# hooman007/ProtoASNet

Hardware: NVIDIA B200
Metric: head_fwd_clips_per_sec (higher is better)
Workload: dtype bf16

## Files before the change

### protoasnet_b200/csrc/head_sm100.cu

```cuda
#include <cstdlib>

#include "head_sm100_shared.cuh"

namespace pasn {
using namespace sm100;

using namespace k1;

namespace {
constexpr int K2_THREADS = 320;
constexpr uint32_t K2_STAGE = 65536;
constexpr uint32_t K2_SM_V = 2 * K2_STAGE;
constexpr uint32_t K2_V_BYTES = PP_MAX * 257 * 4;
constexpr uint32_t K2_SM_MISC = K2_SM_V + 49408;
constexpr uint32_t K2_SM_ORD = K2_SM_MISC + 8192;
constexpr int K2_MAX_ORD = 4096;
constexpr uint32_t K2_SMEM = K2_SM_ORD + 2 * K2_MAX_ORD;

struct K2Params {
  const uint8_t* feimg; const float* osum; const uint8_t* packed; size_t off_w2, off_b2;
  const float* protos; const float* last_layer;
  float* logits; float* sim; float* dist; float* feats;
  const int64_t* labels; const int32_t* proto_class; long long global_offset; unsigned long long* best_key;
  const int* ready;
  int cpc, grid1;
  int* queue;
  int* tile_owner;
  int a_kmajor, l2_hints;
  float* stash;
  int N, P, PP, K, cpt, ntiles;
  int* err;
  int* fault;
  long long* trace;
};
__device__ __forceinline__ long long gtimer_ns() {
  long long t;
  asm volatile("mov.u64 %0, %%globaltimer;" : "=l"(t));
  return t;
}
}
#define K2_TRACE(slot) do { if (p.trace != nullptr && blockIdx.x == 0 && (slot) < 184) p.trace[768 + 16 + (slot)] = gtimer_ns(); } while (0)

__global__ void __launch_bounds__(K2_THREADS, 1) proto_w2_kernel(const K2Params p) {
  extern __shared__ __align__(1024) unsigned char smem[];
  uint64_t* bars = reinterpret_cast<uint64_t*>(smem + K2_SM_MISC);
  uint32_t* tmem_ptr_s = reinterpret_cast<uint32_t*>(smem + K2_SM_MISC + 64);
  volatile int* abort_s = reinterpret_cast<volatile int*>(smem + K2_SM_MISC + 72);
  float* s_vn = reinterpret_cast<float*>(smem + K2_SM_MISC + 128);
  float* s_b2 = reinterpret_cast<float*>(smem + K2_SM_MISC + 512);
  float* s_part = reinterpret_cast<float*>(smem + K2_SM_MISC + 1536);
  float* s_sim = reinterpret_cast<float*>(smem + K2_SM_MISC + 3584);
  unsigned long long* s_key = reinterpret_cast<unsigned long long*>(smem + K2_SM_MISC + 4608);
  uint64_t* tbars = reinterpret_cast<uint64_t*>(smem + K2_SM_MISC + 5632);
  volatile int* s_tile = reinterpret_cast<volatile int*>(smem + K2_SM_MISC + 5696);
  int* s_win = reinterpret_cast<int*>(smem + K2_SM_MISC + 5120);
  float* s_v = reinterpret_cast<float*>(smem + K2_SM_V);

  const int tid = threadIdx.x, warp = tid >> 5, lane = tid & 31;
  Ctx ctx{p.err, abort_s, p.fault, 0};
  if ((smem_u32(smem) & 1023u) != 0) {
    if (tid == 0) atomicCAS(p.err, 0, 901);
    return;
  }
  if (tid == 0) K2_TRACE(0);
  if (tid == 0) {
    *abort_s = 0;
    mbar_init(&bars[0], 1); mbar_init(&bars[1], 1); mbar_init(&bars[2], 1); mbar_init(&bars[3], 1);
    mbar_init(&bars[4], 1); mbar_init(&bars[5], 1); mbar_init(&bars[6], 8); mbar_init(&bars[7], 8);
    for (int i = 0; i < 4; ++i) mbar_init(&tbars[i], 1);
    fence_mbar_init();
  }
  if (warp == 0) tmem_alloc(tmem_ptr_s, 512);
  for (int i = tid; i < DD; i += K2_THREADS) s_b2[i] = reinterpret_cast<const float*>(p.packed + p.off_b2)[i];
  if (tid < p.P) s_key[tid] = p.stash ? (p.best_key[tid] ^ PASN_KEY_SIGN) : PASN_KEY_NONE;
  {
    const float4* src = reinterpret_cast<const float4*>(p.protos);
    const int n4 = p.P * (DD / 4);
#pragma unroll 4
    for (int i = tid; i < n4; i += K2_THREADS) {
      const float4 v = __ldg(src + i);
      float* dst = s_v + ((i * 4) >> 8) * 257 + ((i * 4) & 255);
      dst[0] = v.x; dst[1] = v.y; dst[2] = v.z; dst[3] = v.w;
    }
  }
  __syncthreads();
  for (int pp = warp; pp < p.P; pp += K2_THREADS / 32) {
    float vv = 0.f;
    for (int d = lane; d < DD; d += 32) { const float b = s_v[pp * 257 + d]; vv = fmaf(b, b, vv); }
    vv = warp_sum(vv);
    if (lane == 0) s_vn[pp] = fmaxf(sqrtf(vv), 1e-8f);
  }
  tc_fence_before();
  __syncthreads();
  tc_fence_after();
  const uint32_t tbase = *tmem_ptr_s;
  const uint32_t st_base = smem_u32(smem);
  const bool dynamic = p.ready != nullptr && p.ntiles <= K2_MAX_ORD;
  uint16_t* s_ord = reinterpret_cast<uint16_t*>(smem + K2_SM_ORD);
  if (dynamic) {
    int* s_cnt = reinterpret_cast<int*>(smem);
    const int nslots = p.grid1 * p.cpc;
    const int per = (nslots + K2_THREADS - 1) / K2_THREADS;
    auto emit_tile = [&](int i) -> int {
      const int rnd = i / p.grid1, clip = (i - rnd * p.grid1) * p.cpc + rnd;
      if (clip >= p.N) return -1;
      const int t = clip / p.cpt, c0 = t * p.cpt;
      int c1 = c0 + p.cpt;
      if (c1 > p.N) c1 = p.N;
      int key = 0;
      for (int c = c0; c < c1; ++c) key = max(key, c % p.cpc);
      int first = c0;
      while (first % p.cpc != key) ++first;
      return clip == first ? t : -1;
    };
    const int i0 = tid * per, i1 = min(nslots, i0 + per);
    int cnt = 0;
    for (int i = i0; i < i1; ++i) cnt += emit_tile(i) >= 0 ? 1 : 0;
    s_cnt[tid] = cnt;
    __syncthreads();
    if (tid == 0) {
      int run = 0;
      for (int j = 0; j < K2_THREADS; ++j) { const int c = s_cnt[j]; s_cnt[j] = run; run += c; }
    }
    __syncthreads();
    int pos = s_cnt[tid];
    for (int i = i0; i < i1; ++i) {
      const int t = emit_tile(i);
      if (t >= 0) s_ord[pos++] = (uint16_t)t;
    }
    __syncthreads();
  }
  if (tid == 0) K2_TRACE(1);

  if (warp == 9) {
    if (lane == 0) {
      if (p.ready == nullptr) griddep_wait();
      K2_TRACE(2);
      const uint64_t pol_first = l2_policy_evict_first();
      uint32_t u = 0;
      bool ok = true;
      int dbg_grabs = 0;
      for (int it = 0; ok; ++it) {
        int tile = -1;
        if (dynamic) {
          const int e = atomicAdd(p.queue, 1);
          if (p.trace != nullptr && blockIdx.x == 0 && dbg_grabs < 4) {
            p.trace[768 + 240 + 2 * dbg_grabs] = gtimer_ns();
            p.trace[768 + 240 + 2 * dbg_grabs + 1] = e;
            ++dbg_grabs;
          }
          tile = e < p.ntiles ? (int)s_ord[e] : -1;
        } else {
          tile = (int)blockIdx.x + it * (int)gridDim.x;
          if (tile >= p.ntiles) tile = -1;
        }
        s_tile[it & 3] = tile;
        mbar_arrive(&tbars[it & 3]);
        if (tile < 0) break;
        if (p.tile_owner != nullptr) p.tile_owner[tile] = (int)blockIdx.x;
        const uint8_t* a_src = p.feimg + (size_t)tile * FE_TILE_BYTES;
        if (p.ready != nullptr) {
          int c1 = tile * p.cpt + p.cpt;
          if (c1 > p.N) c1 = p.N;
          const long long t0 = clock64();
          for (int c = tile * p.cpt; c < c1 && ok; ++c) {
            while (ld_acquire_gpu(p.ready + c) < K1_READY_TARGET) {
              __nanosleep(100);
              if (*abort_s || clock64() - t0 > 8000000000ll) { *abort_s = 1; atomicCAS(p.err, 0, 612); if (p.fault) *reinterpret_cast<volatile int*>(p.fault) = 612; ok = false; break; }
            }
          }
          if (!ok) break;
          fence_proxy_async_all();
        }
        K2_TRACE(16 + it * 8 + 7);
        if (p.trace != nullptr && blockIdx.x == 0 && it < 32) p.trace[768 + 200 + it] = tile;
        for (int kc = 0; kc < 4; ++kc, ++u) {
          const uint32_t s = u & 1, ph = (u >> 1) & 1;
          if (!(ok = bwait(&bars[2 + s], ph ^ 1, ctx, 611))) break;
          const uint32_t dst = st_base + s * K2_STAGE;
          mbar_arrive_expect_tx(&bars[s], K2_STAGE);
          if (p.l2_hints) {
            bulk_g2s_hint(dst, a_src + (size_t)kc * 16384, 16384, &bars[s], pol_first);
            bulk_g2s_hint(dst + 16384, a_src + 65536 + (size_t)kc * 16384, 16384, &bars[s], pol_first);
          } else {
            bulk_g2s(dst, a_src + (size_t)kc * 16384, 16384, &bars[s]);
            bulk_g2s(dst + 16384, a_src + 65536 + (size_t)kc * 16384, 16384, &bars[s]);
          }
          bulk_g2s(dst + 32768, p.packed + p.off_w2 + (size_t)kc * 32768, 16384, &bars[s]);
          bulk_g2s(dst + 49152, p.packed + p.off_w2 + (size_t)kc * 32768 + 16384, 16384, &bars[s]);
        }
      }
    }
  } else if (warp == 8) {
    if (elect_one()) {
      const uint32_t idesc = make_idesc_bf16(128, 256, p.a_kmajor ? 0 : 1, 0);
      const uint32_t a_lbo = p.a_kmajor ? 16u : 8192u, a_kstep = p.a_kmajor ? 2u : 128u;
      constexpr uint32_t HI = desc_hi(1024, SWZ_128B);
      const uint32_t bar0 = smem_u32(bars);
      uint32_t u = 0;
      bool ok = true;
      for (int it = 0; ok; ++it) {
        if (!(ok = bwait(&tbars[it & 3], (it >> 2) & 1, ctx, 623))) break;
        if (s_tile[it & 3] < 0) break;
        const uint32_t buf = it & 1;
        if (!(ok = bwait(&bars[6 + buf], ((it >> 1) & 1) ^ 1, ctx, 621))) break;
        tc_fence_after();
        for (int kc = 0; kc < 4 && ok; ++kc, ++u) {
          const uint32_t s = u & 1, ph = (u >> 1) & 1;
          if (!(ok = bwait(&bars[s], ph, ctx, 622))) break;
          K2_TRACE(16 + it * 8 + kc);
          const uint32_t sb = st_base + s * K2_STAGE;
          const uint32_t ah = desc_lo(sb, a_lbo), al = desc_lo(sb + 16384, a_lbo), bd = desc_lo(sb + 32768, 16);
          const uint32_t d = tbase + 256u * buf;
          mma_ss_x(d, ah, HI, bd, HI, idesc, kc ? 1u : 0u);
          mma_ss_x(d, al, HI, bd, HI, idesc, 1u);
#pragma unroll
          for (int k4 = 1; k4 < 4; ++k4) {
            mma_ss_x(d, ah + k4 * a_kstep, HI, bd + k4 * 2, HI, idesc, 1u);
            mma_ss_x(d, al + k4 * a_kstep, HI, bd + k4 * 2, HI, idesc, 1u);
          }
          mma_commit_a(bar0 + 8u * (2 + s));
        }
        if (ok) mma_commit(&bars[4 + buf]);
        K2_TRACE(16 + it * 8 + 4);
      }
    }
  } else {
    const int q = warp & 3, ch = warp >> 2;
    const uint32_t lane_base = (uint32_t)(q * 32) << 16;
    const int r = q * 32 + lane;
    if (p.ready == nullptr) griddep_wait();
    bool ok = true;
    for (int it = 0; ok; ++it) {
      if (!(ok = bwait(&tbars[it & 3], (it >> 2) & 1, ctx, 632))) break;
      const int tile = s_tile[it & 3];
      if (tile < 0) break;
      const uint32_t buf = it & 1;
      const int clip0 = tile * p.cpt;
      int nclip = p.N - clip0;
      if (nclip > p.cpt) nclip = p.cpt;
      const int cl_r = r / p.PP, pp_r = r - cl_r * p.PP;
      const bool rvalid = cl_r < nclip && pp_r < p.P;
      const int cl = rvalid ? cl_r : 0, pp = rvalid ? pp_r : 0;
      const int n = clip0 + cl;
      const float* vrow = s_v + pp * 257 + 128 * ch;
      const float* b2 = s_b2 + 128 * ch;
      float* frow = (p.feats && rvalid) ? p.feats + ((size_t)n * p.P + pp) * DD + 128 * ch : nullptr;
      if (!(ok = bwait(&bars[4 + buf], (it >> 1) & 1, ctx, 631))) break;
      tc_fence_after();
      if (tid == 0) K2_TRACE(16 + it * 8 + 5);
      if (p.ready != nullptr && rvalid) (void)ld_acquire_gpu(p.ready + n);
      const float os = rvalid ? p.osum[(size_t)n * p.P + pp] : 0.f;
      const uint32_t ta = tbase + lane_base + 256u * buf + 128u * ch;
      float ff = 0.f, dot = 0.f;
      uint32_t ra[32], rb[32];
      tmem_ld_x32(ta, ra);
      tmem_ld_wait();
#pragma unroll
      for (int c = 0; c < 4; ++c) {
        uint32_t* cur = (c & 1) ? rb : ra;
        uint32_t* nxt = (c & 1) ? ra : rb;
        if (c < 3) tmem_ld_x32(ta + 32 * (c + 1), *reinterpret_cast<uint32_t(*)[32]>(nxt));
#pragma unroll
        for (int j4 = 0; j4 < 8; ++j4) {
          float f[4];
#pragma unroll
          for (int j = 0; j < 4; ++j) {
            f[j] = fmaf(b2[32 * c + 4 * j4 + j], os, __uint_as_float(cur[4 * j4 + j]));
            ff = fmaf(f[j], f[j], ff);
            dot = fmaf(f[j], vrow[32 * c + 4 * j4 + j], dot);
          }
          if (frow) *reinterpret_cast<float4*>(frow + 32 * c + 4 * j4) = make_float4(f[0], f[1], f[2], f[3]);
        }
        if (c < 3) tmem_ld_wait();
      }
      const bool cap = p.stash != nullptr;
      if (!cap) {
        tc_fence_before();
        __syncwarp();
        if (lane == 0) mbar_arrive(&bars[6 + buf]);
      }
      unsigned long long mykey = PASN_KEY_NONE;
      float* part = s_part + buf * 256;
      float* ssim = s_sim + buf * 128;
      if (ch == 1) { part[2 * r] = dot; part[2 * r + 1] = ff; }
      named_bar_sync(1, 256);
      if (ch == 0) {
        dot += part[2 * r];
        ff += part[2 * r + 1];
        const float nf = fmaxf(sqrtf(ff), 1e-8f);
        const float cosv = dot / (nf * s_vn[pp]);
        const float s = (cosv + 1.0f) / 2.0f;
        const float dd = 1.0f - s;
        ssim[r] = rvalid ? s : 0.f;
        if (rvalid) {
          p.sim[(size_t)n * p.P + pp] = s;
          if (p.dist) p.dist[(size_t)n * p.P + pp] = dd;
          if (p.best_key) {
            const int pc = p.proto_class[pp];
            if (pc < 0 || (long long)pc == p.labels[n]) {
              mykey = pack_key(dd, (uint32_t)(p.global_offset + n));
              atomicMin(&s_key[pp], mykey);
            }
          }
        }
      }
      named_bar_sync(1, 256);
      if (tid < nclip * p.K) {
        const int c2 = tid / p.K, k = tid - c2 * p.K;
        float acc = 0.f;
        for (int qq = 0; qq < p.P; ++qq) acc = fmaf(ssim[c2 * p.PP + qq], p.last_layer[(size_t)k * p.P + qq], acc);
        p.logits[(size_t)(clip0 + c2) * p.K + k] = acc;
      }
      if (cap) {
        if (ch == 0) s_win[r] = (mykey != PASN_KEY_NONE && s_key[pp] == mykey) ? 1 : 0;
        named_bar_sync(1, 256);
        const int win = s_win[r];
        if (__any_sync(0xffffffffu, win != 0)) {
          float* srow = p.stash + ((size_t)blockIdx.x * p.P + pp) * DD + 128 * ch;
#pragma unroll 1
          for (int c = 0; c < 4; ++c) {
            tmem_ld_x32(ta + 32 * c, ra);
            tmem_ld_wait();
            if (win) {
#pragma unroll
              for (int j4 = 0; j4 < 8; ++j4) {
                float f[4];
#pragma unroll
                for (int j = 0; j < 4; ++j) f[j] = fmaf(b2[32 * c + 4 * j4 + j], os, __uint_as_float(ra[4 * j4 + j]));
                *reinterpret_cast<float4*>(srow + 32 * c + 4 * j4) = make_float4(f[0], f[1], f[2], f[3]);
              }
            }
          }
        }
        tc_fence_before();
        __syncwarp();
        if (lane == 0) mbar_arrive(&bars[6 + buf]);
      }
      if (tid == 0) K2_TRACE(16 + it * 8 + 6);
    }
  }
  tc_fence_before();
  __syncthreads();
  if (tid == 0) K2_TRACE(3);
  if (p.best_key && tid < p.P && s_key[tid] != PASN_KEY_NONE) key_atomic_min_global(&p.best_key[tid], s_key[tid]);
  if (warp == 0) tmem_dealloc(tbase, 512);
}

__global__ void pack_weights_kernel(pasn_weights w, int C, int P, int f16, uint8_t* out) {
  const PackedLayout PL = packed_layout(C);
  const int nkc = C / 64;
  const size_t n_l1 = (size_t)2 * nkc * 256 * 64, n_w4 = (size_t)4 * 128 * 64, n_w5 = (size_t)2 * 64 * 64;
  const size_t n_w2 = (size_t)4 * 256 * 64, n_bias = DD + DD + DH, n_b2 = DD;
  const size_t total = n_l1 + n_w4 + n_w5 + n_w2 + n_bias + n_b2;
  for (size_t i = (size_t)blockIdx.x * blockDim.x + threadIdx.x; i < total; i += (size_t)gridDim.x * blockDim.x) {
    size_t j = i;
    if (j < n_l1) {
      const int stage = (int)(j / (256 * 64)), e = (int)(j % (256 * 64));
      const int r = e / 64, k = e % 64, kc = stage >> 1, pass = stage & 1;
      const float v = (pass ? w.addon_w1 : w.occ_w1)[(size_t)r * C + kc * 64 + k];
      uint8_t* dst = out + PL.off_l1 + (size_t)stage * 32768 + off_kmajor_sw128(r, k);
      if (f16) *reinterpret_cast<__half*>(dst) = __float2half_rn(v);
// ... 16 lines not shown
    }
    j -= n_w5;
    if (j < n_w2) {
      const int kc = (int)(j / (256 * 64)), e = (int)(j % (256 * 64)), r = e / 64, k = e % 64;
      *reinterpret_cast<__nv_bfloat16*>(out + PL.off_w2 + (size_t)kc * 32768 + off_kmajor_sw128(r, k)) =
          __float2bfloat16_rn(w.addon_w2[(size_t)r * DD + kc * 64 + k]);
      continue;
    }
    j -= n_w2;
    if (j < n_bias) {
      float v;
      if (j < DD) v = w.occ_b1[j];
      else if (j < 2 * DD) v = w.addon_b1[j - DD];
      else v = w.occ_b2[j - 2 * DD];
      reinterpret_cast<float*>(out + PL.off_bias)[j] = round_bf16(v);
      continue;
    }
    j -= n_bias;
    reinterpret_cast<float*>(out + PL.off_b2)[j] = round_bf16(w.addon_b2[j]);
  }
}

__global__ void push_capture_stash_kernel(const unsigned long long* __restrict__ best_key, int P, long long offset, int N,
                                          int cpt, int grid2, const int* __restrict__ tile_owner, const float* __restrict__ stash,
                                          float* __restrict__ best_vec) {
  const int pp = blockIdx.x;
  const unsigned long long key = best_key[pp] ^ PASN_KEY_SIGN;
  if (key == PASN_KEY_NONE) return;
  const long long idx = (long long)(key & 0xFFFFFFFFull);
  if (idx < offset || idx >= offset + N) return;
  const int tile = (int)((idx - offset) / cpt);
  const int cta = tile_owner != nullptr ? tile_owner[tile] : tile % grid2;
  const float* src = stash + ((size_t)cta * P + pp) * DD;
  for (int d = threadIdx.x; d < DD; d += blockDim.x) best_vec[(size_t)pp * DD + d] = src[d];
}

static long long* g_trace = nullptr;
void sm100_set_trace(void* dev_buf) { g_trace = reinterpret_cast<long long*>(dev_buf); }
static int g_k1_variant = -1;
void sm100_set_k1_variant(int variant) { g_k1_variant = variant; }

bool sm100_supported(const pasn_dims& d) {
  const bool half = d.dtype == PASN_BF16 || d.dtype == PASN_F16;
  if (d.layout != PASN_LAYOUT_NCS && !(d.layout == PASN_LAYOUT_NSC && half)) return false;
  if (!half && !(d.dtype == PASN_F32 && d.path == PASN_PATH_TCGEN05)) return false;
  if (d.D != DD) return false;
  if (d.C % 64 != 0 || d.C < 64 || d.C > 1024) return false;
  if (d.P < 1 || d.P > PP_MAX) return false;
  if (d.S % 4 != 0 || d.S < TILE_M) return false;
  return true;
}

size_t sm100_packed_bytes(const pasn_dims& d) { return packed_layout(d.C).total; }

static inline int k2_ppad(const pasn_dims& d) {
  const int p8 = (d.P + 7) / 8 * 8;
  return p8 <= 16 ? 16 : p8 <= 32 ? 32 : p8 <= 40 ? 40 : 48;
}
static inline int split_groups(const pasn_dims& d) {
  if (d.N <= 0 || d.N > 74) return 1;
  static const int allow = [] { const char* e = getenv("PASN_NO_SPLIT"); return (e && atoi(e) != 0) ? 0 : 1; }();
  if (!allow) return 1;
  int best = 1;
  for (int g = 2; g <= d.S / TILE_M; ++g) {
    if (d.S % g != 0) continue;
    const int sv = d.S / g;
    if (sv < TILE_M || sv % 4 != 0) continue;
    if ((long long)d.N * g > 148) break;
    best = g;
  }
  return best;
}
constexpr int K2_MAX_GRID = 160;
struct WsLayout {
  int G, Nv, Sv, tiles2;
  size_t off_osum, off_err, off_ready, off_owner, off_stash, off_featsv, off_fe, off_simv, off_logv, total;
};
static inline WsLayout ws_layout(const pasn_dims& d) {
  WsLayout L;
  L.G = split_groups(d);
  L.Nv = d.N * L.G;
  L.Sv = d.S / L.G;
  L.tiles2 = ceil_div(L.Nv, TILE_M / k2_ppad(d));
  size_t o = (size_t)L.tiles2 * FE_TILE_BYTES;
  L.off_osum = o; o += align_up((size_t)L.Nv * d.P * 4, 256);
  L.off_err = o; o += 256;
  L.off_ready = o; o += align_up((size_t)L.Nv * 4, 256);
  L.off_owner = o; o += align_up((size_t)L.tiles2 * 4, 256);
  L.off_stash = o; o += align_up((size_t)K2_MAX_GRID * d.P * DD * 4, 256);
  L.off_featsv = L.off_fe = L.off_simv = L.off_logv = o;
  if (L.G > 1) {
    L.off_featsv = o; o += align_up((size_t)L.Nv * d.P * DD * 4, 256);
    L.off_fe = o; o += align_up((size_t)d.N * d.P * DD * 4, 256);
    L.off_simv = o; o += align_up((size_t)L.Nv * d.P * 4, 256);
    L.off_logv = o; o += align_up((size_t)L.Nv * d.K * 4, 256);
  }
  L.total = o;
  return L;
}

size_t sm100_workspace_bytes(const pasn_dims& d) { return ws_layout(d).total; }

__global__ void sum_groups_kernel(const float* __restrict__ fev, float* __restrict__ fe, int N, int G, int PD) {
  const long long i = (long long)blockIdx.x * blockDim.x + threadIdx.x;
  if (i >= (long long)N * PD) return;
  const long long n = i / PD, r = i - n * PD;
  float a = 0.f;
  for (int g = 0; g < G; ++g) a += fev[((size_t)n * G + g) * PD + r];
  fe[i] = a;
}

// ... 2 lines not shown
  pack_weights_kernel<<<148 * 4, 256, 0, st>>>(w, d.C, d.P, d.dtype == PASN_F16 ? 1 : 0, reinterpret_cast<uint8_t*>(packed));
  PASN_LAUNCH_CHECK();
  count_launch();
  return PASN_OK;
}

int sm100_head_forward(const void* feat, const pasn_weights& w, const void* packed, const pasn_dims& d, float* logits,
                       float* sim, void* occ, float* feats, float* dist, const pasn_push_args* push, void* ws,
                       size_t ws_bytes, cudaStream_t st) {
  if (!sm100_supported(d)) return PASN_ERR_UNSUPPORTED;
  if (ws_bytes < sm100_workspace_bytes(d)) return PASN_ERR_WORKSPACE;
  if (((uintptr_t)feat & 15) != 0 || ((uintptr_t)packed & 15) != 0 || ((uintptr_t)ws & 15) != 0) return PASN_ERR_ALIGN;
  static bool attr_done = false;
  if (!attr_done) {
    if (cudaFuncSetAttribute(proto_w2_kernel, cudaFuncAttributeMaxDynamicSharedMemorySize, (int)K2_SMEM) != cudaSuccess)
      return PASN_ERR_CUDA;
    attr_done = true;
  }
  const WsLayout L = ws_layout(d);
  char* wsp = reinterpret_cast<char*>(ws);
  uint8_t* feimg = reinterpret_cast<uint8_t*>(wsp);
  float* osum = reinterpret_cast<float*>(wsp + L.off_osum);
  int* err = reinterpret_cast<int*>(wsp + L.off_err);
  int* ready = reinterpret_cast<int*>(wsp + L.off_ready);

  static const int num_sms = [] {
    int dev = 0, n = 0;
    if (cudaGetDevice(&dev) != cudaSuccess || cudaDeviceGetAttribute(&n, cudaDevAttrMultiProcessorCount, dev) != cudaSuccess || n <= 0) n = 148;
    return n > K2_MAX_GRID ? K2_MAX_GRID : n;
  }();
  K1Params k1{};
  k1.f32_in = d.dtype == PASN_F32;
  k1.f16_in = d.dtype == PASN_F16;
  k1.nsc = d.layout == PASN_LAYOUT_NSC;
  k1.feat = reinterpret_cast<const __nv_bfloat16*>(feat);
  k1.feat32 = reinterpret_cast<const float*>(feat);
  k1.packed = reinterpret_cast<const uint8_t*>(packed);
  k1.occ = k1.f32_in ? nullptr : reinterpret_cast<__nv_bfloat16*>(occ);
  k1.occ32 = k1.f32_in ? reinterpret_cast<float*>(occ) : nullptr;
  k1.feimg = feimg; k1.osum = osum;
  k1.N = L.Nv; k1.C = d.C; k1.P = d.P; k1.S = L.Sv; k1.nkc = d.C / 64;
  k1.G = L.G; k1.SR = d.S;
  k1.clips_per_cta = ceil_div(L.Nv, num_sms);
  k1.cpt = TILE_M / k2_ppad(d);
  k1.err = err;
  k1.fault = fault_word();
  k1.trace = g_trace;
  { const char* e = getenv("PASN_DBG_SKIP"); k1.dbg_skip = e ? atoi(e) : 0; }
  static const int flush_kmajor = [] { const char* e = getenv("PASN_FLUSH_KMAJOR"); return (PASN_K1_EXPERIMENTS && e) ? atoi(e) : 1; }();
  static const int l2_hints = [] { const char* e = getenv("PASN_L2_HINTS"); return (PASN_K1_EXPERIMENTS && e) ? atoi(e) : 1; }();
  k1.flush_kmajor = flush_kmajor; k1.l2_hints = l2_hints;
  static const int x_drain = [] { const char* e = getenv("PASN_X_DRAIN"); return e ? atoi(e) : 0; }();
  k1.x_drain = x_drain;
  static const int spin = [] { const char* e = getenv("PASN_K1_SPIN"); return e ? atoi(e) : 0; }();
  k1.spin = spin;
  static const int flush_sleep = [] { const char* e = getenv("PASN_FLUSH_SLEEP"); return e ? atoi(e) : 0; }();
  k1.flush_sleep = flush_sleep;
  static const int k2_early = [] { const char* e = getenv("PASN_K2_EARLY"); return (PASN_K1_EXPERIMENTS && e) ? atoi(e) : 0; }();
  k1.ready = k2_early ? ready : nullptr;
  static const int dbg_sync = [] { const char* e = getenv("PASN_DEBUG_SYNC"); return e ? atoi(e) : 0; }();
  if ((k2_early || dbg_sync) && cudaMemsetAsync(err, 0, 256 + (size_t)L.Nv * 4, st) != cudaSuccess) return PASN_ERR_CUDA;
  const int grid1 = ceil_div(L.Nv, k1.clips_per_cta);
  const int ppad = (d.P + 7) / 8 * 8;
  static const int env_variant = [] {
    const char* e = getenv("PASN_K1_PHASES");
    const int v = e ? atoi(e) : 1;
    return v == 2 ? 2 : 1;
  }();
  const int variant = g_k1_variant == 2 ? 2 : (g_k1_variant == 1 ? 1 : env_variant);
  k1.phases = variant;
  main_kernel_begin(st);
  const int rc = launch_k1_two_phase(k1, ppad, grid1, st);
  if (rc) return rc;
  main_kernel_end(st);
  count_launch();
  if (logits == nullptr) return PASN_OK;

  const PackedLayout PL = packed_layout(d.C);
  K2Params k2{};
  k2.feimg = feimg; k2.osum = osum; k2.packed = k1.packed; k2.off_w2 = PL.off_w2; k2.off_b2 = PL.off_b2;
  k2.protos = w.prototypes; k2.last_layer = w.last_layer;
  const bool split = L.G > 1;
  float* featsv = reinterpret_cast<float*>(wsp + L.off_featsv);
  k2.logits = split ? reinterpret_cast<float*>(wsp + L.off_logv) : logits;
  k2.sim = split ? reinterpret_cast<float*>(wsp + L.off_simv) : sim;
  k2.dist = split ? nullptr : dist;
  k2.feats = split ? featsv : feats;
  k2.labels = (push && !split) ? push->labels : nullptr;
  k2.proto_class = (push && !split) ? push->proto_class : nullptr;
  k2.global_offset = (push && !split) ? (long long)push->global_offset : 0;
  k2.best_key = (push && !split) ? reinterpret_cast<unsigned long long*>(push->best_key) : nullptr;
  k2.stash = (push && !split && push->best_vec) ? reinterpret_cast<float*>(wsp + L.off_stash) : nullptr;
  k2.N = L.Nv; k2.P = d.P; k2.K = d.K;
  k2.cpt = TILE_M / k2_ppad(d);
  k2.PP = k2_ppad(d);
  k2.ntiles = L.tiles2;
  k2.err = err;
  k2.fault = k1.fault;
  k2.trace = g_trace;
  k2.a_kmajor = flush_kmajor; k2.l2_hints = l2_hints;
  k2.ready = k2_early ? ready : nullptr; k2.cpc = k1.clips_per_cta; k2.grid1 = grid1;
  k2.queue = err + 1;
  k2.tile_owner = k2_early ? reinterpret_cast<int*>(wsp + L.off_owner) : nullptr;
  const int grid2 = k2.ntiles < num_sms ? k2.ntiles : num_sms;
  {
    cudaLaunchConfig_t cfg{};
    cfg.gridDim = dim3(grid2); cfg.blockDim = dim3(K2_THREADS); cfg.dynamicSmemBytes = K2_SMEM; cfg.stream = st;
    cudaLaunchAttribute at[1];
    at[0].id = cudaLaunchAttributeProgrammaticStreamSerialization;
    at[0].val.programmaticStreamSerializationAllowed = 1;
    cfg.attrs = at; cfg.numAttrs = 1;
    if (cudaLaunchKernelEx(&cfg, proto_w2_kernel, k2) != cudaSuccess) return PASN_ERR_CUDA;
  }
  PASN_LAUNCH_CHECK();
  count_launch();
  if (k2.stash) {
    push_capture_stash_kernel<<<d.P, 128, 0, st>>>(k2.best_key, d.P, k2.global_offset, L.Nv, k2.cpt, grid2, k2.tile_owner, k2.stash,
                                                   push->best_vec);
    PASN_LAUNCH_CHECK();
    count_launch();
  }
  if (split) {
    float* fe = feats ? feats : reinterpret_cast<float*>(wsp + L.off_fe);
    const long long tot = (long long)d.N * d.P * DD;
    sum_groups_kernel<<<(unsigned)((tot + 255) / 256), 256, 0, st>>>(featsv, fe, d.N, L.G, d.P * DD);
    PASN_LAUNCH_CHECK();
    count_launch();
    const int rc2 = launch_proto_stage(fe, w.prototypes, w.last_layer, d.N, d.P, DD, d.K, logits, sim, dist, push, st);
    if (rc2) return rc2;
  }
  return PASN_OK;
}

int sm100_occurrence_only(const void* feat, const pasn_weights& w, const void* packed, const pasn_dims& d, void* occ, void* ws,
                          size_t ws_bytes, cudaStream_t st) {
  return sm100_head_forward(feat, w, packed, d, nullptr, nullptr, occ, nullptr, nullptr, nullptr, ws, ws_bytes, st);
}

int sm100_last_error(const void* ws, const pasn_dims& d, cudaStream_t st) {
  const char* wsp = reinterpret_cast<const char*>(ws);
  const int* err = reinterpret_cast<const int*>(wsp + ws_layout(d).off_err);
// ... 8 lines not shown
```

### protoasnet_b200/csrc/head_sm100_k1.cu

```cuda
#include <cstdlib>

#include "head_sm100_shared.cuh"

namespace pasn {
using namespace sm100;
using namespace k1;

namespace {

#ifndef PASN_XSLOTS
#define PASN_XSLOTS 4
#endif
#ifndef PASN_WSLOTS
#define PASN_WSLOTS 3
#endif
constexpr int XSLOTS = PASN_XSLOTS, WSLOTS = PASN_WSLOTS, XDEPTH = XSLOTS - 1;
constexpr uint32_t XSLOT_BYTES = 16384, WSLOT_BYTES = 32768;
constexpr int K1_WARPS = 16, K1_THREADS = K1_WARPS * 32;
constexpr int W_MMA = 0, W_WPROD = 1, W_TAIL = 2, W_OCC = 3, W_X0 = 4, W_EPI0 = 8;
constexpr uint32_t SM_X = 0;
constexpr uint32_t SM_W = SM_X + XSLOTS * XSLOT_BYTES;
constexpr uint32_t SM_OS = SM_W + WSLOTS * WSLOT_BYTES;
constexpr uint32_t OS_BYTES_MAX = TILE_M * 2 * PP_MAX * 2;
constexpr uint32_t SM_BIAS = SM_OS + OS_BYTES_MAX;
// ... 548 lines not shown
#pragma unroll 8
          for (int tok = 0; tok < TILE_M; ++tok)
            a += __bfloat162float(*reinterpret_cast<const __nv_bfloat16*>(os + off_mnmajor_nosw(n0, tok, NPOOL)));
          s0[slot] = a;
        }
        if (lane + 32 < PP) {
          float a = 0.f;
#pragma unroll 8
          for (int tok = 0; tok < TILE_M; ++tok)
            a += __bfloat162float(*reinterpret_cast<const __nv_bfloat16*>(os + off_mnmajor_nosw(n1, tok, NPOOL)));
          s1[slot] = a;
        }
      }
      __syncwarp();
      if (lane == 0) mbar_arrive(&bars[B_OSEMPTY]);
      const int last_tok = min(tile * TILE_M + TILE_M - 1, ntok - 1);
      const int last_clip = last_tok / S;
      acc0 += s0[0]; acc1 += s1[0];
      if (last_clip > first_clip) {
        if (lane < p.P) p.osum[(size_t)(c_begin + first_clip) * p.P + lane] = acc0;
        if (lane + 32 < p.P) p.osum[(size_t)(c_begin + first_clip) * p.P + lane + 32] = acc1;
        acc0 = s0[1]; acc1 = s1[1];
        __syncwarp();
        if (PASN_K1_EXPERIMENTS && p.ready != nullptr && lane == 0) red_release_gpu_add(p.ready + c_begin + first_clip, 1);
      }
      if ((last_tok + 1) % S == 0) {
        if (lane < p.P) p.osum[(size_t)(c_begin + last_clip) * p.P + lane] = acc0;
        if (lane + 32 < p.P) p.osum[(size_t)(c_begin + last_clip) * p.P + lane + 32] = acc1;
        acc0 = acc1 = 0.f;
        __syncwarp();
        if (PASN_K1_EXPERIMENTS && p.ready != nullptr && lane == 0) red_release_gpu_add(p.ready + c_begin + last_clip, 1);
      }
    }
  } else if (warp >= W_EPI0) {
    const int q = warp & 3, hh = (warp - W_EPI0) >> 2;
    const uint32_t lane_base = (uint32_t)(q * 32) << 16;
    const uint32_t tl = tbase + lane_base;
    const int tok = q * 32 + lane;
    const int d = 128 * hh + tok;
    const float b1d = sb1[d];
    const bool tr = TRACE && warp == W_EPI0 && lane == 0;
    float facc[PP];
#pragma unroll
    for (int i = 0; i < PP; ++i) facc[i] = 0.f;
    bool ok = true;
    const uint64_t pol_last = l2_policy_evict_last();

    auto h1t_convert = [&](int tile) -> bool {
      if (!bwait(&bars[B_ADONE], tile & 1, ctx, 507)) return false;
      tc_fence_after();
      if (tr) K1_TRACE(1, tile, 7);
      uint32_t ra[32], rb[32], pk[16];
      const int c0 = hh ? 3 : 0, dc = hh ? -1 : 1;
      const uint32_t src = COL_AT + 128u * hh, dst = hh ? COL_H1T1 : COL_H1T0;
// ... 133 lines not shown
        const uint32_t fe = tl + ((hh && !two_phase) ? 0u : COL_FE);
        uint32_t nb[PP];
        {
          uint32_t a[PP];
#pragma unroll
          for (int g = 0; g < PP / 8; ++g) tmem_ld_x8(fe + 8 * g, *reinterpret_cast<uint32_t(*)[8]>(&a[8 * g]));
          if (boundary) {
#pragma unroll
            for (int g = 0; g < PP / 8; ++g) tmem_ld_x8(fe + PP + 8 * g, *reinterpret_cast<uint32_t(*)[8]>(&nb[8 * g]));
          }
          tmem_ld_wait();
#pragma unroll
          for (int j = 0; j < PP; ++j) facc[j] += __uint_as_float(a[j]);
        }
        tc_fence_before();
        __syncwarp();
        if (lane == 0) mbar_arrive(&bars[hh ? B_ABFREE : B_FEFREE0]);
        if (tr) K1_TRACE(1, tile, 10);
#pragma unroll 1
        for (int rep = 0; rep < 2; ++rep) {
          const bool flush = rep == 0 ? boundary : ends;
          if (!flush) continue;
          if (dbg_skip & 8) {
            if (PASN_K1_EXPERIMENTS && p.ready != nullptr && lane == 0) red_release_gpu_add(p.ready + c_begin + (rep == 0 ? first_clip : last_clip), 1);
            if (rep == 0) {
#pragma unroll
              for (int j = 0; j < PP; ++j) facc[j] = __uint_as_float(nb[j]);
            } else {
#pragma unroll
              for (int j = 0; j < PP; ++j) facc[j] = 0.f;
            }
            continue;
          }
          const int clip = c_begin + (rep == 0 ? first_clip : last_clip);
          const int tile2 = clip / p.cpt;
          const int rowb = (clip - tile2 * p.cpt) * PP;
          uint8_t* img = p.feimg + (size_t)tile2 * FE_TILE_BYTES + (size_t)(d >> 6) * 16384;
          if (flush_kmajor) {
#pragma unroll
            for (int j = 0; j < PP; ++j) {
              const float v = facc[j];
              const __nv_bfloat16 h = __float2bfloat16_rn(v);
              const __nv_bfloat16 l = __float2bfloat16_rn(v - __bfloat162float(h));
              const uint32_t off = off_kmajor_sw128(rowb + j, d & 63);
              if (l2_hints) {
                st_global_u16_hint(img + off, __bfloat16_as_ushort(h), pol_last);
                st_global_u16_hint(img + 65536 + off, __bfloat16_as_ushort(l), pol_last);
              } else {
                *reinterpret_cast<__nv_bfloat16*>(img + off) = h;
                *reinterpret_cast<__nv_bfloat16*>(img + 65536 + off) = l;
              }
              if (flush_sleep && (j & 3) == 3) __nanosleep(flush_sleep);
            }
          } else {
#pragma unroll
            for (int c = 0; c < PP / 8; ++c) {
              uint32_t hi4[4], lo4[4];
#pragma unroll
              for (int j = 0; j < 4; ++j) {
                const float v0 = facc[8 * c + 2 * j], v1 = facc[8 * c + 2 * j + 1];
                const float h0 = round_bf16(v0), h1 = round_bf16(v1);
                hi4[j] = pack_bf16x2(h0, h1);
                lo4[j] = pack_bf16x2(v0 - h0, v1 - h1);
              }
              const uint32_t off = off_mnmajor_sw128(rowb + 8 * c, d & 63, 8192);
              *reinterpret_cast<uint4*>(img + off) = make_uint4(hi4[0], hi4[1], hi4[2], hi4[3]);
              *reinterpret_cast<uint4*>(img + 65536 + off) = make_uint4(lo4[0], lo4[1], lo4[2], lo4[3]);
            }
          }
          __syncwarp();
          if (PASN_K1_EXPERIMENTS && p.ready != nullptr && lane == 0) red_release_gpu_add(p.ready + clip, 1);
          if (rep == 0) {
#pragma unroll
            for (int j = 0; j < PP; ++j) facc[j] = __uint_as_float(nb[j]);
          } else {
#pragma unroll
            for (int j = 0; j < PP; ++j) facc[j] = 0.f;
          }
        }
      }
    }
  }

  tc_fence_before();
  __syncthreads();
  if (warp == 0) tmem_dealloc(tbase, 512);
  if constexpr (TRACE) {
    if (tid == 0 && p.trace != nullptr && blockIdx.x == 0) {
      long long t;
      asm volatile("mov.u64 %0, %%globaltimer;" : "=l"(t));
      p.trace[768 + 1] = t;
    }
  }
}
// ... 32 lines not shown
```

### protoasnet_b200/csrc/head_sm100_shared.cuh

```cuda
#pragma once
#include "common.cuh"
#include "sm100_prims.cuh"

namespace pasn {
namespace k1 {
using namespace sm100;

constexpr int TILE_M = 128;
constexpr int DD = 256;
constexpr int DH = DD / 2;
constexpr int PP_MAX = 48;
constexpr int K1_READY_TARGET = 9;
constexpr uint32_t FE_TILE_BYTES = 131072;

struct PackedLayout {
  size_t off_l1, off_w4, off_w5, off_bias, off_w2, off_b2, total;
};
__host__ __device__ inline PackedLayout packed_layout(int C) {
  PackedLayout L;
  const int nkc = C / 64;
  L.off_l1 = 0;
  L.off_w4 = (size_t)2 * nkc * 32768;
  L.off_w5 = L.off_w4 + 65536;
  L.off_bias = L.off_w5 + 16384;
  L.off_w2 = (L.off_bias + (DD + DD + DH) * 4 + 1023) / 1024 * 1024;
  L.off_b2 = L.off_w2 + 4 * 32768;
  L.total = L.off_b2 + DD * 4;
  return L;
}

struct K1Params {
  const __nv_bfloat16* feat;
  const float* feat32;
  float* occ32;
  int f32_in;
  int nsc;
  const uint8_t* packed;
  __nv_bfloat16* occ;
  uint8_t* feimg;
  float* osum;
  int N, C, P, S, nkc, clips_per_cta, cpt;
  int G, SR;
  int* err;
  int* fault;
  long long* trace;
  int phases;
  int dbg_skip;
  int flush_kmajor;
  int* ready;
  int l2_hints;
  int flush_sleep;
  int x_drain;
  int spin;
  int f16_in;
};

#ifndef PASN_K1_EXPERIMENTS
#define PASN_K1_EXPERIMENTS 0
#endif

struct Ctx {
  int* err;
  volatile int* abort_s;
  int* fault;
  int spin;
};

static __device__ __noinline__ bool bwait_slow(uint64_t* bar, uint32_t parity, int* err, volatile int* abort_s, int* fault, int code,
                                               int spin) {
  const long long t0 = clock64();
  const bool poll = (spin >> (code / 100)) & 1;
  while (!(poll ? mbar_test_wait(bar, parity) : mbar_try_wait(bar, parity))) {
// ... 44 lines not shown
```

Before: 6.081 million.

## Split K2 pipeline into separate W2/A slots and prefetch weights before grid dependency

Restructures the K2 load pipeline from two 64KB stages holding both A tiles and W2 weights into five 32KB slots, where W2 and feature-image chunks are loaded separately. The first W2 chunks are issued before griddepcontrol.wait so weight loads can overlap the tail of the preceding kernel. Removes the experimental dynamic tile queue and ready-flag early-start path in favor of static round-robin tiles. Also vectorizes prototype stores with a padded stride and float4 bias/prototype reads, and unrolls the logits loop. W2 is still reloaded per tile, so total bytes moved stay about the same.

New measurement: 6.107 million, median of 6. Within noise of the previous version (+0.4%).

```diff
diff --git a/protoasnet_b200/csrc/head_sm100.cu b/protoasnet_b200/csrc/head_sm100.cu
--- a/protoasnet_b200/csrc/head_sm100.cu
+++ b/protoasnet_b200/csrc/head_sm100.cu
@@ -9,23 +9,18 @@
 
 namespace {
 constexpr int K2_THREADS = 320;
-constexpr uint32_t K2_STAGE = 65536;
-constexpr uint32_t K2_SM_V = 2 * K2_STAGE;
-constexpr uint32_t K2_V_BYTES = PP_MAX * 257 * 4;
-constexpr uint32_t K2_SM_MISC = K2_SM_V + 49408;
-constexpr uint32_t K2_SM_ORD = K2_SM_MISC + 8192;
-constexpr int K2_MAX_ORD = 4096;
-constexpr uint32_t K2_SMEM = K2_SM_ORD + 2 * K2_MAX_ORD;
+constexpr uint32_t K2_SLOT = 32768;
+constexpr int K2_NSLOT = 5;
+constexpr int K2_VSTRIDE = 260;
+constexpr uint32_t K2_SM_V = K2_NSLOT * K2_SLOT;
+constexpr uint32_t K2_SM_MISC = K2_SM_V + PP_MAX * K2_VSTRIDE * 4;
+constexpr uint32_t K2_SMEM = K2_SM_MISC + 8192;
 
 struct K2Params {
   const uint8_t* feimg; const float* osum; const uint8_t* packed; size_t off_w2, off_b2;
   const float* protos; const float* last_layer;
   float* logits; float* sim; float* dist; float* feats;
   const int64_t* labels; const int32_t* proto_class; long long global_offset; unsigned long long* best_key;
-  const int* ready;
-  int cpc, grid1;
-  int* queue;
-  int* tile_owner;
   int a_kmajor, l2_hints;
   float* stash;
   int N, P, PP, K, cpt, ntiles;
@@ -44,17 +39,19 @@
 __global__ void __launch_bounds__(K2_THREADS, 1) proto_w2_kernel(const K2Params p) {
   extern __shared__ __align__(1024) unsigned char smem[];
   uint64_t* bars = reinterpret_cast<uint64_t*>(smem + K2_SM_MISC);
-  uint32_t* tmem_ptr_s = reinterpret_cast<uint32_t*>(smem + K2_SM_MISC + 64);
-  volatile int* abort_s = reinterpret_cast<volatile int*>(smem + K2_SM_MISC + 72);
-  float* s_vn = reinterpret_cast<float*>(smem + K2_SM_MISC + 128);
+  uint32_t* tmem_ptr_s = reinterpret_cast<uint32_t*>(smem + K2_SM_MISC + 128);
+  volatile int* abort_s = reinterpret_cast<volatile int*>(smem + K2_SM_MISC + 136);
+  float* s_vn = reinterpret_cast<float*>(smem + K2_SM_MISC + 256);
   float* s_b2 = reinterpret_cast<float*>(smem + K2_SM_MISC + 512);
   float* s_part = reinterpret_cast<float*>(smem + K2_SM_MISC + 1536);
   float* s_sim = reinterpret_cast<float*>(smem + K2_SM_MISC + 3584);
   unsigned long long* s_key = reinterpret_cast<unsigned long long*>(smem + K2_SM_MISC + 4608);
-  uint64_t* tbars = reinterpret_cast<uint64_t*>(smem + K2_SM_MISC + 5632);
-  volatile int* s_tile = reinterpret_cast<volatile int*>(smem + K2_SM_MISC + 5696);
   int* s_win = reinterpret_cast<int*>(smem + K2_SM_MISC + 5120);
   float* s_v = reinterpret_cast<float*>(smem + K2_SM_V);
+  uint64_t* full = bars;
+  uint64_t* empty = bars + K2_NSLOT;
+  uint64_t* accfull = bars + 2 * K2_NSLOT;
+  uint64_t* accempty = accfull + 2;
 
   const int tid = threadIdx.x, warp = tid >> 5, lane = tid & 31;
   Ctx ctx{p.err, abort_s, p.fault, 0};
@@ -65,9 +62,8 @@
   if (tid == 0) K2_TRACE(0);
   if (tid == 0) {
     *abort_s = 0;
-    mbar_init(&bars[0], 1); mbar_init(&bars[1], 1); mbar_init(&bars[2], 1); mbar_init(&bars[3], 1);
-    mbar_init(&bars[4], 1); mbar_init(&bars[5], 1); mbar_init(&bars[6], 8); mbar_init(&bars[7], 8);
-    for (int i = 0; i < 4; ++i) mbar_init(&tbars[i], 1);
+    for (int i = 0; i < K2_NSLOT; ++i) { mbar_init(&full[i], 1); mbar_init(&empty[i], 1); }
+    mbar_init(&accfull[0], 1); mbar_init(&accfull[1], 1); mbar_init(&accempty[0], 8); mbar_init(&accempty[1], 8);
     fence_mbar_init();
   }
   if (warp == 0) tmem_alloc(tmem_ptr_s, 512);
@@ -79,14 +75,13 @@
 #pragma unroll 4
     for (int i = tid; i < n4; i += K2_THREADS) {
       const float4 v = __ldg(src + i);
-      float* dst = s_v + ((i * 4) >> 8) * 257 + ((i * 4) & 255);
-      dst[0] = v.x; dst[1] = v.y; dst[2] = v.z; dst[3] = v.w;
+      *reinterpret_cast<float4*>(s_v + ((i * 4) >> 8) * K2_VSTRIDE + ((i * 4) & 255)) = v;
     }
   }
   __syncthreads();
   for (int pp = warp; pp < p.P; pp += K2_THREADS / 32) {
     float vv = 0.f;
-    for (int d = lane; d < DD; d += 32) { const float b = s_v[pp * 257 + d]; vv = fmaf(b, b, vv); }
+    for (int d = lane; d < DD; d += 32) { const float b = s_v[pp * K2_VSTRIDE + d]; vv = fmaf(b, b, vv); }
     vv = warp_sum(vv);
     if (lane == 0) s_vn[pp] = fmaxf(sqrtf(vv), 1e-8f);
   }
@@ -95,99 +90,39 @@
   tc_fence_after();
   const uint32_t tbase = *tmem_ptr_s;
   const uint32_t st_base = smem_u32(smem);
-  const bool dynamic = p.ready != nullptr && p.ntiles <= K2_MAX_ORD;
-  uint16_t* s_ord = reinterpret_cast<uint16_t*>(smem + K2_SM_ORD);
-  if (dynamic) {
-    int* s_cnt = reinterpret_cast<int*>(smem);
-    const int nslots = p.grid1 * p.cpc;
-    const int per = (nslots + K2_THREADS - 1) / K2_THREADS;
-    auto emit_tile = [&](int i) -> int {
-      const int rnd = i / p.grid1, clip = (i - rnd * p.grid1) * p.cpc + rnd;
-      if (clip >= p.N) return -1;
-      const int t = clip / p.cpt, c0 = t * p.cpt;
-      int c1 = c0 + p.cpt;
-      if (c1 > p.N) c1 = p.N;
-      int key = 0;
-      for (int c = c0; c < c1; ++c) key = max(key, c % p.cpc);
-      int first = c0;
-      while (first % p.cpc != key) ++first;
-      return clip == first ? t : -1;
-    };
-    const int i0 = tid * per, i1 = min(nslots, i0 + per);
-    int cnt = 0;
-    for (int i = i0; i < i1; ++i) cnt += emit_tile(i) >= 0 ? 1 : 0;
-    s_cnt[tid] = cnt;
-    __syncthreads();
-    if (tid == 0) {
-      int run = 0;
-      for (int j = 0; j < K2_THREADS; ++j) { const int c = s_cnt[j]; s_cnt[j] = run; run += c; }
-    }
-    __syncthreads();
-    int pos = s_cnt[tid];
-    for (int i = i0; i < i1; ++i) {
-      const int t = emit_tile(i);
-      if (t >= 0) s_ord[pos++] = (uint16_t)t;
-    }
-    __syncthreads();
-  }
+  const int ntile_cta = p.ntiles > (int)blockIdx.x ? (p.ntiles - 1 - (int)blockIdx.x) / (int)gridDim.x + 1 : 0;
   if (tid == 0) K2_TRACE(1);
 
   if (warp == 9) {
     if (lane == 0) {
-      if (p.ready == nullptr) griddep_wait();
+      const uint32_t nent = 8u * (uint32_t)ntile_cta;
+      const uint8_t* w2 = p.packed + p.off_w2;
+      for (uint32_t e = 0; e < K2_NSLOT && e < nent; e += 2) {
+        mbar_arrive_expect_tx(&full[e], K2_SLOT);
+        bulk_g2s(st_base + e * K2_SLOT, w2 + (size_t)(e >> 1) * K2_SLOT, K2_SLOT, &full[e]);
+      }
+      griddep_wait();
       K2_TRACE(2);
       const uint64_t pol_first = l2_policy_evict_first();
-      uint32_t u = 0;
-      bool ok = true;
-      int dbg_grabs = 0;
-      for (int it = 0; ok; ++it) {
-        int tile = -1;
-        if (dynamic) {
-          const int e = atomicAdd(p.queue, 1);
-          if (p.trace != nullptr && blockIdx.x == 0 && dbg_grabs < 4) {
-            p.trace[768 + 240 + 2 * dbg_grabs] = gtimer_ns();
-            p.trace[768 + 240 + 2 * dbg_grabs + 1] = e;
-            ++dbg_grabs;
+      for (uint32_t e = 0; e < nent; ++e) {
+        if (e < K2_NSLOT && (e & 1) == 0) continue;
+        const uint32_t s = e % K2_NSLOT, ph = (e / K2_NSLOT) & 1;
+        if (!bwait(&empty[s], ph ^ 1, ctx, 611)) break;
+        const uint32_t dst = st_base + s * K2_SLOT;
+        const int kc = (int)((e >> 1) & 3);
+        mbar_arrive_expect_tx(&full[s], K2_SLOT);
+        if ((e & 1) == 0) {
+          bulk_g2s(dst, w2 + (size_t)kc * K2_SLOT, K2_SLOT, &full[s]);
+        } else {
+          const int tile = (int)blockIdx.x + (int)(e >> 3) * (int)gridDim.x;
+          const uint8_t* a_src = p.feimg + (size_t)tile * FE_TILE_BYTES + (size_t)kc * 16384;
+          if (p.l2_hints) {
+            bulk_g2s_hint(dst, a_src, 16384, &full[s], pol_first);
+            bulk_g2s_hint(dst + 16384, a_src + 65536, 16384, &full[s], pol_first);
+          } else {
+            bulk_g2s(dst, a_src, 16384, &full[s]);
+            bulk_g2s(dst + 16384, a_src + 65536, 16384, &full[s]);
           }
-          tile = e < p.ntiles ? (int)s_ord[e] : -1;
-        } else {
-          tile = (int)blockIdx.x + it * (int)gridDim.x;
-          if (tile >= p.ntiles) tile = -1;
-        }
-        s_tile[it & 3] = tile;
-        mbar_arrive(&tbars[it & 3]);
-        if (tile < 0) break;
-        if (p.tile_owner != nullptr) p.tile_owner[tile] = (int)blockIdx.x;
-        const uint8_t* a_src = p.feimg + (size_t)tile * FE_TILE_BYTES;
-        if (p.ready != nullptr) {
-          int c1 = tile * p.cpt + p.cpt;
-          if (c1 > p.N) c1 = p.N;
-          const long long t0 = clock64();
-          for (int c = tile * p.cpt; c < c1 && ok; ++c) {
-            while (ld_acquire_gpu(p.ready + c) < K1_READY_TARGET) {
-              __nanosleep(100);
-              if (*abort_s || clock64() - t0 > 8000000000ll) { *abort_s = 1; atomicCAS(p.err, 0, 612); if (p.fault) *reinterpret_cast<volatile int*>(p.fault) = 612; ok = false; break; }
-            }
-          }
-          if (!ok) break;
-          fence_proxy_async_all();
-        }
-        K2_TRACE(16 + it * 8 + 7);
-        if (p.trace != nullptr && blockIdx.x == 0 && it < 32) p.trace[768 + 200 + it] = tile;
-        for (int kc = 0; kc < 4; ++kc, ++u) {
-          const uint32_t s = u & 1, ph = (u >> 1) & 1;
-          if (!(ok = bwait(&bars[2 + s], ph ^ 1, ctx, 611))) break;
-          const uint32_t dst = st_base + s * K2_STAGE;
-          mbar_arrive_expect_tx(&bars[s], K2_STAGE);
-          if (p.l2_hints) {
-            bulk_g2s_hint(dst, a_src + (size_t)kc * 16384, 16384, &bars[s], pol_first);
-            bulk_g2s_hint(dst + 16384, a_src + 65536 + (size_t)kc * 16384, 16384, &bars[s], pol_first);
-          } else {
-            bulk_g2s(dst, a_src + (size_t)kc * 16384, 16384, &bars[s]);
-            bulk_g2s(dst + 16384, a_src + 65536 + (size_t)kc * 16384, 16384, &bars[s]);
-          }
-          bulk_g2s(dst + 32768, p.packed + p.off_w2 + (size_t)kc * 32768, 16384, &bars[s]);
-          bulk_g2s(dst + 49152, p.packed + p.off_w2 + (size_t)kc * 32768 + 16384, 16384, &bars[s]);
         }
       }
     }
@@ -197,20 +132,19 @@
       const uint32_t a_lbo = p.a_kmajor ? 16u : 8192u, a_kstep = p.a_kmajor ? 2u : 128u;
       constexpr uint32_t HI = desc_hi(1024, SWZ_128B);
       const uint32_t bar0 = smem_u32(bars);
-      uint32_t u = 0;
+      uint32_t e = 0;
       bool ok = true;
-      for (int it = 0; ok; ++it) {
-        if (!(ok = bwait(&tbars[it & 3], (it >> 2) & 1, ctx, 623))) break;
-        if (s_tile[it & 3] < 0) break;
+      for (int it = 0; it < ntile_cta && ok; ++it) {
         const uint32_t buf = it & 1;
-        if (!(ok = bwait(&bars[6 + buf], ((it >> 1) & 1) ^ 1, ctx, 621))) break;
+        if (!(ok = bwait(&accempty[buf], ((it >> 1) & 1) ^ 1, ctx, 621))) break;
         tc_fence_after();
-        for (int kc = 0; kc < 4 && ok; ++kc, ++u) {
-          const uint32_t s = u & 1, ph = (u >> 1) & 1;
-          if (!(ok = bwait(&bars[s], ph, ctx, 622))) break;
-          K2_TRACE(16 + it * 8 + kc);
-          const uint32_t sb = st_base + s * K2_STAGE;
-          const uint32_t ah = desc_lo(sb, a_lbo), al = desc_lo(sb + 16384, a_lbo), bd = desc_lo(sb + 32768, 16);
+        for (int kc = 0; kc < 4 && ok; ++kc, e += 2) {
+          const uint32_t sw = e % K2_NSLOT, sa = (e + 1) % K2_NSLOT;
+          if (!(ok = bwait(&full[sw], (e / K2_NSLOT) & 1, ctx, 622))) break;
+          if (!(ok = bwait(&full[sa], ((e + 1) / K2_NSLOT) & 1, ctx, 622))) break;
+          if (it < 16) K2_TRACE(16 + it * 8 + kc);
+          const uint32_t sb = st_base + sa * K2_SLOT;
+          const uint32_t ah = desc_lo(sb, a_lbo), al = desc_lo(sb + 16384, a_lbo), bd = desc_lo(st_base + sw * K2_SLOT, 16);
           const uint32_t d = tbase + 256u * buf;
           mma_ss_x(d, ah, HI, bd, HI, idesc, kc ? 1u : 0u);
           mma_ss_x(d, al, HI, bd, HI, idesc, 1u);
@@ -219,38 +153,36 @@
             mma_ss_x(d, ah + k4 * a_kstep, HI, bd + k4 * 2, HI, idesc, 1u);
             mma_ss_x(d, al + k4 * a_kstep, HI, bd + k4 * 2, HI, idesc, 1u);
           }
-          mma_commit_a(bar0 + 8u * (2 + s));
+          mma_commit_a(bar0 + 8u * (K2_NSLOT + sw));
+          mma_commit_a(bar0 + 8u * (K2_NSLOT + sa));
         }
-        if (ok) mma_commit(&bars[4 + buf]);
-        K2_TRACE(16 + it * 8 + 4);
+        if (ok) mma_commit(&accfull[buf]);
+        if (it < 16) K2_TRACE(16 + it * 8 + 4);
       }
     }
   } else {
     const int q = warp & 3, ch = warp >> 2;
     const uint32_t lane_base = (uint32_t)(q * 32) << 16;
     const int r = q * 32 + lane;
-    if (p.ready == nullptr) griddep_wait();
+    const int cl_r = r / p.PP, pp_r = r - cl_r * p.PP;
+    const float* b2 = s_b2 + 128 * ch;
+    griddep_wait();
     bool ok = true;
-    for (int it = 0; ok; ++it) {
-      if (!(ok = bwait(&tbars[it & 3], (it >> 2) & 1, ctx, 632))) break;
-      const int tile = s_tile[it & 3];
-      if (tile < 0) break;
+    for (int it = 0; it < ntile_cta && ok; ++it) {
+      const int tile = (int)blockIdx.x + it * (int)gridDim.x;
       const uint32_t buf = it & 1;
       const int clip0 = tile * p.cpt;
       int nclip = p.N - clip0;
       if (nclip > p.cpt) nclip = p.cpt;
-      const int cl_r = r / p.PP, pp_r = r - cl_r * p.PP;
       const bool rvalid = cl_r < nclip && pp_r < p.P;
       const int cl = rvalid ? cl_r : 0, pp = rvalid ? pp_r : 0;
       const int n = clip0 + cl;
-      const float* vrow = s_v + pp * 257 + 128 * ch;
-      const float* b2 = s_b2 + 128 * ch;
+      const float* vrow = s_v + pp * K2_VSTRIDE + 128 * ch;
       float* frow = (p.feats && rvalid) ? p.feats + ((size_t)n * p.P + pp) * DD + 128 * ch : nullptr;
-      if (!(ok = bwait(&bars[4 + buf], (it >> 1) & 1, ctx, 631))) break;
+      const float os = rvalid ? p.osum[(size_t)n * p.P + pp] : 0.f;
+      if (!(ok = bwait(&accfull[buf], (it >> 1) & 1, ctx, 631))) break;
       tc_fence_after();
-      if (tid == 0) K2_TRACE(16 + it * 8 + 5);
-      if (p.ready != nullptr && rvalid) (void)ld_acquire_gpu(p.ready + n);
-      const float os = rvalid ? p.osum[(size_t)n * p.P + pp] : 0.f;
+      if (tid == 0 && it < 16) K2_TRACE(16 + it * 8 + 5);
       const uint32_t ta = tbase + lane_base + 256u * buf + 128u * ch;
       float ff = 0.f, dot = 0.f;
       uint32_t ra[32], rb[32];
@@ -263,12 +195,15 @@
         if (c < 3) tmem_ld_x32(ta + 32 * (c + 1), *reinterpret_cast<uint32_t(*)[32]>(nxt));
 #pragma unroll
         for (int j4 = 0; j4 < 8; ++j4) {
+          const float4 bb = *reinterpret_cast<const float4*>(b2 + 32 * c + 4 * j4);
+          const float4 vv = *reinterpret_cast<const float4*>(vrow + 32 * c + 4 * j4);
+          const float bv[4] = {bb.x, bb.y, bb.z, bb.w}, pv[4] = {vv.x, vv.y, vv.z, vv.w};
           float f[4];
 #pragma unroll
           for (int j = 0; j < 4; ++j) {
-            f[j] = fmaf(b2[32 * c + 4 * j4 + j], os, __uint_as_float(cur[4 * j4 + j]));
+            f[j] = fmaf(bv[j], os, __uint_as_float(cur[4 * j4 + j]));
             ff = fmaf(f[j], f[j], ff);
-            dot = fmaf(f[j], vrow[32 * c + 4 * j4 + j], dot);
+            dot = fmaf(f[j], pv[j], dot);
           }
           if (frow) *reinterpret_cast<float4*>(frow + 32 * c + 4 * j4) = make_float4(f[0], f[1], f[2], f[3]);
         }
@@ -278,7 +213,7 @@
       if (!cap) {
         tc_fence_before();
         __syncwarp();
-        if (lane == 0) mbar_arrive(&bars[6 + buf]);
+        if (lane == 0) mbar_arrive(&accempty[buf]);
       }
       unsigned long long mykey = PASN_KEY_NONE;
       float* part = s_part + buf * 256;
@@ -308,8 +243,11 @@
       named_bar_sync(1, 256);
       if (tid < nclip * p.K) {
         const int c2 = tid / p.K, k = tid - c2 * p.K;
+        const float* srow = ssim + c2 * p.PP;
+        const float* lrow = p.last_layer + (size_t)k * p.P;
         float acc = 0.f;
-        for (int qq = 0; qq < p.P; ++qq) acc = fmaf(ssim[c2 * p.PP + qq], p.last_layer[(size_t)k * p.P + qq], acc);
+#pragma unroll 8
+        for (int qq = 0; qq < p.P; ++qq) acc = fmaf(srow[qq], __ldg(lrow + qq), acc);
         p.logits[(size_t)(clip0 + c2) * p.K + k] = acc;
       }
       if (cap) {
@@ -335,9 +273,9 @@
         }
         tc_fence_before();
         __syncwarp();
-        if (lane == 0) mbar_arrive(&bars[6 + buf]);
-      }
-      if (tid == 0) K2_TRACE(16 + it * 8 + 6);
+        if (lane == 0) mbar_arrive(&accempty[buf]);
+      }
+      if (tid == 0 && it < 16) K2_TRACE(16 + it * 8 + 6);
     }
   }
   tc_fence_before();
@@ -400,16 +338,14 @@
 }
 
 __global__ void push_capture_stash_kernel(const unsigned long long* __restrict__ best_key, int P, long long offset, int N,
-                                          int cpt, int grid2, const int* __restrict__ tile_owner, const float* __restrict__ stash,
-                                          float* __restrict__ best_vec) {
+                                          int cpt, int grid2, const float* __restrict__ stash, float* __restrict__ best_vec) {
   const int pp = blockIdx.x;
   const unsigned long long key = best_key[pp] ^ PASN_KEY_SIGN;
   if (key == PASN_KEY_NONE) return;
   const long long idx = (long long)(key & 0xFFFFFFFFull);
   if (idx < offset || idx >= offset + N) return;
   const int tile = (int)((idx - offset) / cpt);
-  const int cta = tile_owner != nullptr ? tile_owner[tile] : tile % grid2;
-  const float* src = stash + ((size_t)cta * P + pp) * DD;
+  const float* src = stash + ((size_t)(tile % grid2) * P + pp) * DD;
   for (int d = threadIdx.x; d < DD; d += blockDim.x) best_vec[(size_t)pp * DD + d] = src[d];
 }
 
@@ -452,7 +388,7 @@
 constexpr int K2_MAX_GRID = 160;
 struct WsLayout {
   int G, Nv, Sv, tiles2;
-  size_t off_osum, off_err, off_ready, off_owner, off_stash, off_featsv, off_fe, off_simv, off_logv, total;
+  size_t off_osum, off_err, off_stash, off_featsv, off_fe, off_simv, off_logv, total;
 };
 static inline WsLayout ws_layout(const pasn_dims& d) {
   WsLayout L;
@@ -463,8 +399,6 @@
   size_t o = (size_t)L.tiles2 * FE_TILE_BYTES;
   L.off_osum = o; o += align_up((size_t)L.Nv * d.P * 4, 256);
   L.off_err = o; o += 256;
-  L.off_ready = o; o += align_up((size_t)L.Nv * 4, 256);
-  L.off_owner = o; o += align_up((size_t)L.tiles2 * 4, 256);
   L.off_stash = o; o += align_up((size_t)K2_MAX_GRID * d.P * DD * 4, 256);
   L.off_featsv = L.off_fe = L.off_simv = L.off_logv = o;
   if (L.G > 1) {
@@ -513,7 +447,6 @@
   uint8_t* feimg = reinterpret_cast<uint8_t*>(wsp);
   float* osum = reinterpret_cast<float*>(wsp + L.off_osum);
   int* err = reinterpret_cast<int*>(wsp + L.off_err);
-  int* ready = reinterpret_cast<int*>(wsp + L.off_ready);
 
   static const int num_sms = [] {
     int dev = 0, n = 0;
@@ -547,10 +480,8 @@
   k1.spin = spin;
   static const int flush_sleep = [] { const char* e = getenv("PASN_FLUSH_SLEEP"); return e ? atoi(e) : 0; }();
   k1.flush_sleep = flush_sleep;
-  static const int k2_early = [] { const char* e = getenv("PASN_K2_EARLY"); return (PASN_K1_EXPERIMENTS && e) ? atoi(e) : 0; }();
-  k1.ready = k2_early ? ready : nullptr;
   static const int dbg_sync = [] { const char* e = getenv("PASN_DEBUG_SYNC"); return e ? atoi(e) : 0; }();
-  if ((k2_early || dbg_sync) && cudaMemsetAsync(err, 0, 256 + (size_t)L.Nv * 4, st) != cudaSuccess) return PASN_ERR_CUDA;
+  if (dbg_sync && cudaMemsetAsync(err, 0, 256, st) != cudaSuccess) return PASN_ERR_CUDA;
   const int grid1 = ceil_div(L.Nv, k1.clips_per_cta);
   const int ppad = (d.P + 7) / 8 * 8;
   static const int env_variant = [] {
@@ -590,9 +521,6 @@
   k2.fault = k1.fault;
   k2.trace = g_trace;
   k2.a_kmajor = flush_kmajor; k2.l2_hints = l2_hints;
-  k2.ready = k2_early ? ready : nullptr; k2.cpc = k1.clips_per_cta; k2.grid1 = grid1;
-  k2.queue = err + 1;
-  k2.tile_owner = k2_early ? reinterpret_cast<int*>(wsp + L.off_owner) : nullptr;
   const int grid2 = k2.ntiles < num_sms ? k2.ntiles : num_sms;
   {
     cudaLaunchConfig_t cfg{};
@@ -606,8 +534,7 @@
   PASN_LAUNCH_CHECK();
   count_launch();
   if (k2.stash) {
-    push_capture_stash_kernel<<<d.P, 128, 0, st>>>(k2.best_key, d.P, k2.global_offset, L.Nv, k2.cpt, grid2, k2.tile_owner, k2.stash,
-                                                   push->best_vec);
+    push_capture_stash_kernel<<<d.P, 128, 0, st>>>(k2.best_key, d.P, k2.global_offset, L.Nv, k2.cpt, grid2, k2.stash, push->best_vec);
     PASN_LAUNCH_CHECK();
     count_launch();
   }
diff --git a/protoasnet_b200/csrc/head_sm100_k1.cu b/protoasnet_b200/csrc/head_sm100_k1.cu
--- a/protoasnet_b200/csrc/head_sm100_k1.cu
+++ b/protoasnet_b200/csrc/head_sm100_k1.cu
@@ -594,14 +594,12 @@
         if (lane + 32 < p.P) p.osum[(size_t)(c_begin + first_clip) * p.P + lane + 32] = acc1;
         acc0 = s0[1]; acc1 = s1[1];
         __syncwarp();
-        if (PASN_K1_EXPERIMENTS && p.ready != nullptr && lane == 0) red_release_gpu_add(p.ready + c_begin + first_clip, 1);
       }
       if ((last_tok + 1) % S == 0) {
         if (lane < p.P) p.osum[(size_t)(c_begin + last_clip) * p.P + lane] = acc0;
         if (lane + 32 < p.P) p.osum[(size_t)(c_begin + last_clip) * p.P + lane + 32] = acc1;
         acc0 = acc1 = 0.f;
         __syncwarp();
-        if (PASN_K1_EXPERIMENTS && p.ready != nullptr && lane == 0) red_release_gpu_add(p.ready + c_begin + last_clip, 1);
       }
     }
   } else if (warp >= W_EPI0) {
@@ -781,7 +779,6 @@
           const bool flush = rep == 0 ? boundary : ends;
           if (!flush) continue;
           if (dbg_skip & 8) {
-            if (PASN_K1_EXPERIMENTS && p.ready != nullptr && lane == 0) red_release_gpu_add(p.ready + c_begin + (rep == 0 ? first_clip : last_clip), 1);
             if (rep == 0) {
 #pragma unroll
               for (int j = 0; j < PP; ++j) facc[j] = __uint_as_float(nb[j]);
@@ -828,7 +825,6 @@
             }
           }
           __syncwarp();
-          if (PASN_K1_EXPERIMENTS && p.ready != nullptr && lane == 0) red_release_gpu_add(p.ready + clip, 1);
           if (rep == 0) {
 #pragma unroll
             for (int j = 0; j < PP; ++j) facc[j] = __uint_as_float(nb[j]);
diff --git a/protoasnet_b200/csrc/head_sm100_shared.cuh b/protoasnet_b200/csrc/head_sm100_shared.cuh
--- a/protoasnet_b200/csrc/head_sm100_shared.cuh
+++ b/protoasnet_b200/csrc/head_sm100_shared.cuh
@@ -10,7 +10,6 @@
 constexpr int DD = 256;
 constexpr int DH = DD / 2;
 constexpr int PP_MAX = 48;
-constexpr int K1_READY_TARGET = 9;
 constexpr uint32_t FE_TILE_BYTES = 131072;
 
 struct PackedLayout {
@@ -47,7 +46,6 @@
   int phases;
   int dbg_skip;
   int flush_kmajor;
-  int* ready;
   int l2_hints;
   int flush_sleep;
   int x_drain;
```
